# LiChaiUSTC/Speech-enhancement-based-on-a-maximum-likelihood-criterion

Measured on AMD Instinct MI355X. Metric: training frames/sec (128-frame minibatch), higher is better.
Workload: dtype f32

## Files before the change

### speech-enhancement-based-on-a-maximum-likelihood-criterion_amd/csrc/engine.hip

```cpp
#include <hip/hip_runtime.h>
#include <hip/hip_ext.h>

#include <dlfcn.h>
#include <math.h>
#include <stdarg.h>
#include <stdio.h>
#include <stdlib.h>
#include <string.h>

#include <functional>
#include <mutex>
#include <string>
#include <vector>

#include "../../include/mlggd.h"
#include "kernels.hip.h"
#include "spectral.hip.h"
#include "score.hip.h"

static thread_local char g_err[1024] = "";
static int fail(int code, const char *fmt, ...) {
    va_list ap;
    va_start(ap, fmt);
    vsnprintf(g_err, sizeof(g_err), fmt, ap);
// ... 127 lines not shown
    int device = 0;
    hipStream_t stream = nullptr, comm_stream = nullptr;
    hipStream_t dw_stream = nullptr;
    hipEvent_t ev_dx[MLGGD_MAXLAYER] = {0}, ev_upd = nullptr;
    int two_streams = 0;

    float *W[MLGGD_MAXLAYER] = {0}, *dW[MLGGD_MAXLAYER] = {0};
    float *bias[MLGGD_MAXLAYER] = {0}, *dbias[MLGGD_MAXLAYER] = {0};
    float *G[MLGGD_MAXLAYER] = {0}, *gb[MLGGD_MAXLAYER] = {0};
    float *gb_all = nullptr;
    size_t gb_all_count = 0;
    float *Gpre[MLGGD_MAXLAYER] = {0}, *gbpre = nullptr, *colsum_tot = nullptr;
    float *Yt[MLGGD_MAXLAYER] = {0}, *Y[MLGGD_MAXLAYER] = {0};
    float *dEdXt[MLGGD_MAXLAYER] = {0}, *dEdX[MLGGD_MAXLAYER] = {0};
    float *slab = nullptr, *outT = nullptr, *eT = nullptr, *pT = nullptr, *colsum = nullptr, *scalefactor = nullptr;
    int S_out = 1;
    float *chunk_in = nullptr, *chunk_targ = nullptr, *chunk_out = nullptr;
    int cv_device = 0;
    double *cv_partial = nullptr;
    size_t cv_partial_cap = 0;
    size_t chunk_cap = 0, out_cap = 0;
    int chunk_frames = 0;
    float *raw_feat = nullptr, *raw_targ = nullptr, *in_bunch = nullptr;
    float *in_bunch_buf[2] = {nullptr, nullptr};
    int *first_frame = nullptr;
    size_t raw_cap = 0, first_cap = 0;
    struct RawSet {
        float *feat = nullptr, *targ = nullptr;
        int *first = nullptr;
        size_t raw_cap = 0, first_cap = 0;
        hipEvent_t last_use = nullptr;
    } raw[2];
    int raw_cur = 0;
    hipStream_t copy_stream = nullptr;
    struct WsBuf {
        void *p = nullptr;
        size_t cap = 0;
    };
    struct WavesWs {
        WsBuf wave, lps, X, blk, out_i, out_f, lps_den, norm, frame_off, out_off, wave_off, utt_of;
        WsBuf clean, Xc, fstat, sframes, scores;
        std::vector<int32_t> h_frame_off, h_utt_of;
        std::vector<long long> h_out_off, h_wave_off;
        std::vector<float> h_norm;
        std::vector<float> h_scores;
        int lookup_table = 0;
    } ww;
    bool indexed = false;
    int fdim = 0, toff = 0, raw_frames = 0;
    unsigned step_counter = 0;
    int fwd_pipe = 4, dx_pipe = 4;
    int tile64 = 1, n_cus = 256;
    int fwd_nw = 4, dx_nw = 4, dw_tile = 1, dw_persist = 1, dwp_per_cu = 2, dw_merge = 1, loss_fuse = 1, tile_map = 0, stage_ahead = 1;

    int world = 1, rank = 0;
    int dp_mode = 0;
    int shard_rows[MLGGD_MAXLAYER] = {0};
    int dp_a2a = 0;
    std::vector<float *> Ysrc[MLGGD_MAXLAYER];
    hipEvent_t ev_W[MLGGD_MAXLAYER] = {0}, ev_dw_done = nullptr;
    bool ev_W_pending[MLGGD_MAXLAYER] = {false};
    bool fake_world = false;
    float *Yall[MLGGD_MAXLAYER] = {0}, *dEdXall[MLGGD_MAXLAYER] = {0};
    bool keep_ranks = false;
    std::vector<float *> snap_x, snap_out, snap_y[MLGGD_MAXLAYER], snap_dedx[MLGGD_MAXLAYER];
    hipEvent_t ev_ready = nullptr, ev_gathered = nullptr;
    int dp_fine = 1;
    hipEvent_t ev_layer[MLGGD_MAXLAYER] = {0};
    int dp_mainline = 1;
    bool comm_after_dw = false;
    RcclComm comm = nullptr;
    RcclComm stat_comm = nullptr;
    int ar_shard = 1;
    hipEvent_t ev_grad[MLGGD_MAXLAYER] = {0}, ev_red[MLGGD_MAXLAYER] = {0}, ev_bias = nullptr, ev_bias_red = nullptr;

    hipEvent_t ev_t0 = nullptr, ev_t1 = nullptr;
    int last_steps = 0;
    bool timing_valid = false;
    int prof_class = -1, prof_layer = 0, prof_stride = 1;
    std::vector<hipEvent_t> prof_ev;
    size_t prof_used = 0, prof_cap = 0;
    hipEvent_t *prof_attach = nullptr;
    bool prof_attached = false;
    hipEvent_t stop_ev_next = nullptr;
    bool stop_ev_attached = false;
    int dp_stopev = 1;
    double prof_flops = 0, prof_bytes = 0;

    int stamp_class = -1, stamp_layer = 0, stamp_blocks = 0;
    long long *stamp_buf = nullptr;
    size_t stamp_cap = 0;

    struct DwpTable {
        DwpJobs key;
        bool fused;
        int grid;
        DwpDesc *dev;
    };
    std::vector<DwpTable> dwp_tables;
    std::vector<void *> allocs;
    std::vector<const void *> lds_attr_done;
};

static long long *stamps_for(mlggd_engine *e, int cls, int layer, int blocks) {
    if (e->stamp_class != cls || e->stamp_layer != layer || !e->stamp_buf) return nullptr;
    if ((size_t)blocks * 8 > e->stamp_cap) return nullptr;
// ... 756 lines not shown
    CHK(launch_check("k_loss_err"));
    const float *colsum_in = nullptr;
    if (ML == 1 && cs == CS_GIVEN) {
        colsum_in = e->colsum_tot;
    } else if (ML == 1 && cs != CS_LOCAL) {
        hipLaunchKernelGGL(k_colsum, dim3(e->Dp / 32), dim3(256), 0, e->stream, e->pT, B, Bp, e->colsum);
        CHK(launch_check("k_colsum"));
        if (cs == CS_ACCUMULATE) {
            hipLaunchKernelGGL(k_accum, dim3(1), dim3(256), 0, e->stream, e->colsum_tot,
                               first_acc ? (const float *)nullptr : (const float *)e->colsum_tot, (const float *)e->colsum,
                               (size_t)e->Dp);
            return launch_check("k_accum");
        }
        NCCLCHK(g_rccl.AllReduce(e->colsum, e->colsum, (size_t)e->Dp, 7, 0, e->stat_comm ? e->stat_comm : e->comm, e->stream));
        colsum_in = e->colsum;
    }
    if (cs == CS_ACCUMULATE) return MLGGD_OK;
    CHK(ensure_lds(e, k_loss_grad, LOSS_LDS_MAX));
    hipLaunchKernelGGL(k_loss_grad, dim3(n_loss), dim3(256), lds_grad, e->stream, e->eT, e->pT, colsum_in, B, e->D, e->Dp, Bp,
                       e->cfg.shapefactor, ML, nf, inv_n, e->scalefactor, e->dEdXt[L - 1], e->dEdX[L - 1], b_tiles);
    return launch_check("k_loss_grad");
}

static int run_dx(mlggd_engine *e, int l) {
    const int Kp = e->lsp[l - 1], b_tiles = e->Bp / 32;
    ProfScope ps(e, KC_DX, l);
    DxArgs xa = dx_args(e, l);
    if (dx64_used(e, l)) {
        xa.k_tiles = Kp / 64;
        xa.b_tiles = e->Bp / 64;
        xa.b_shift = log2_or_minus1(xa.b_tiles);
        const size_t lds = t64_lds_floats() * sizeof(float);
        CHK(ensure_lds(e, k_dx64, lds));
        launch_timed(e, k_dx64, dim3(xa.k_tiles * xa.b_tiles), dim3(256), lds, e->stream, xa);
        return launch_check("k_dx64");
    }
    long long *st = stamps_for(e, KC_DX, l, (Kp / 32) * b_tiles);
#define LAUNCH_DX(NW, PIPE)                                                                                  \
    {                                                                                                        \
        const size_t lds = dx_lds_floats<NW, PIPE>() * sizeof(float);                                        \
        CHK(ensure_lds(e, k_dx<NW, PIPE>, lds));                                                             \
        launch_timed(e, k_dx<NW, PIPE>, dim3((Kp / 32) * b_tiles), dim3(64 * NW), lds, e->stream, xa, st);      \
    }
    const bool dma = e->dx_pipe == 4 && (Kp / 32) * b_tiles <= 256;
    if (e->dx_nw == 8 && e->dx_pipe) LAUNCH_DX(8, 1)
    else if (e->dx_nw == 8) LAUNCH_DX(8, 0)
    else if (dma) LAUNCH_DX(4, 4)
    else if (e->dx_pipe) LAUNCH_DX(4, 1)
    else LAUNCH_DX(4, 0)
#undef LAUNCH_DX
    return launch_check("k_dx");
}

static int launch_dw_layer(mlggd_engine *e, int l, const float *in_rows, bool fused, float nf, hipStream_t st) {
    const int Kp = e->lsp[l - 1], Np = e->lsp[l];
    const long tiles128 = (long)((Kp + 127) / 128) * ((Np + 127) / 128);
    const bool big = e->dw_tile == 0 ? tiles128 >= 192 : e->dw_tile == 2;
    ProfScope ps(e, KC_DW, l, st);
    if (dwp_usable(e)) return launch_dwp(e, dwp_jobs(e, l, l, in_rows, nf), fused, st, l);
    if (big) return launch_dw<2>(e, l, in_rows, fused, nf, st);
    return launch_dw<1>(e, l, in_rows, fused, nf, st);
}

static int launch_accum(float *dst, const float *a, const float *b, size_t n, hipStream_t st) {
    const size_t blocks = (n + 255) / 256;
    hipLaunchKernelGGL(k_accum, dim3((unsigned)(blocks > 2048 ? 2048 : blocks)), dim3(256), 0, st, dst, a, b, n);
    return launch_check("k_accum");
}

static size_t y_count(const mlggd_engine *e, int l) {
    return e->dp_a2a ? (size_t)e->world * e->Bp * e->shard_rows[l + 1] * 64 : (size_t)e->Bp * e->lsp[l];
}
static int keep_alloc(mlggd_engine *e) {
    if (!e->keep_ranks || !e->fake_world || !e->snap_x.empty()) return MLGGD_OK;
    for (int r = 0; r + 1 < e->world; r++) {
        float *p = nullptr;
        CHK(dev_alloc(e, &p, y_count(e, 0)));
        e->snap_x.push_back(p);
        CHK(dev_alloc(e, &p, (size_t)e->Dp * e->Bp));
        e->snap_out.push_back(p);
        for (int l = 1; l < e->L; l++) {
            if (l < e->L - 1) {
                CHK(dev_alloc(e, &p, y_count(e, l)));
                e->snap_y[l].push_back(p);
            }
            CHK(dev_alloc(e, &p, (size_t)e->Bp * e->lsp[l]));
            e->snap_dedx[l].push_back(p);
        }
    }
    HIPCHK(hipStreamSynchronize(e->stream));
    return MLGGD_OK;
}
static int keep_snapshot(mlggd_engine *e, int r, const float *in_rows) {
    auto cp = [&](float *dst, const float *src, size_t count) -> int {
        HIPCHK(hipMemcpyAsync(dst, src, count * sizeof(float), hipMemcpyDeviceToDevice, e->stream));
        return MLGGD_OK;
    };
    CHK(cp(e->snap_x[r], in_rows, y_count(e, 0)));
    CHK(cp(e->snap_out[r], e->outT, (size_t)e->Dp * e->Bp));
    for (int l = 1; l < e->L; l++) {
        if (l < e->L - 1) CHK(cp(e->snap_y[l][r], e->Y[l], y_count(e, l)));
        CHK(cp(e->snap_dedx[l][r], e->dEdX[l], (size_t)e->Bp * e->lsp[l]));
    }
    return MLGGD_OK;
}

// ... 21 lines not shown
            };
            if (e->dp_a2a) {
                for (int l = 0; l < L - 1; l++) {
                    const size_t all = (size_t)e->world * Bp * e->shard_rows[l + 1] * 64;
                    HIPCHK(hipMemcpyAsync(e->Ysrc[l][r], l == 0 ? in_rows : e->Y[l], all * sizeof(float), hipMemcpyDeviceToDevice, e->stream));
                }
            } else {
                CHK(put(in_rows, e->Yall[0], (size_t)Bp * e->lsp[0]));
                for (int l = 1; l < L - 1; l++) CHK(put(e->Y[l], e->Yall[l], (size_t)Bp * e->lsp[l]));
            }
            for (int l = 1; l < L; l++) CHK(put(e->dEdX[l], e->dEdXall[l], (size_t)Bp * e->lsp[l]));
        } else {
            for (int l = L - 1; l >= 1; l--) {
                CHK(launch_dw_layer(e, l, in_rows, false, nf, e->stream));
                CHK(launch_accum(e->Gpre[l], r == 0 ? nullptr : e->Gpre[l], e->G[l], (size_t)e->lsp[l - 1] * e->lsp[l], e->stream));
            }
            CHK(launch_accum(e->gbpre, r == 0 ? nullptr : e->gbpre, e->gb_all, e->gb_all_count, e->stream));
        }
    }
    return MLGGD_OK;
}

static int run_step(mlggd_engine *e, int sample0, bool prestaged = false, const Bunch *next = nullptr) {
    const int L = e->L, B = e->B, Bp = e->Bp;
    e->stop_ev_next = nullptr;
    e->stop_ev_attached = false;
    const bool dp = e->comm != nullptr || e->fake_world;
    const bool gather = dp && e->dp_mode >= 1;
    const int n_global = B * e->world;
    const float nf = (float)n_global;
    const float inv_n = 1.0f / n_global;
    const int ML = e->cfg.MLflag;
    if (e->fake_world) {
        CHK(fake_world_prepass(e, sample0, nf, inv_n));
        sample0 += (e->world - 1) * B;
    }
    const Bunch bn = bunch_at(e, sample0);
    RoctxRange step_range("mlggd step");

    const bool fine = gather && e->dp_mode == 1 && e->dp_fine != 0;
    {
        RoctxRange r("forward");
        CHK(run_forward(e, bn, B, true, prestaged,
                        gather ? (GATHER_INPUT | (ML != 1 ? (fine ? GATHER_HIDDEN_EACH : GATHER_HIDDEN) : 0)) : 0));
    }
    const float *in_rows = bunch_rows(e, bn);
    StageArgs sa;
    memset(&sa, 0, sizeof(sa));
    int n_stage = 0;
    if (next) {
        sa = stage_args(e, *next, B, in_bunch_other(e));
        n_stage = stage_blocks(e);
    }
    {
        RoctxRange r("loss (+ staging of the next minibatch)");
        CHK(run_loss(e, bn, nf, inv_n, !dp ? CS_LOCAL : e->fake_world ? CS_GIVEN : CS_ALLREDUCE, false, sa, n_stage));
    }
    RoctxRange back_range("backward: dX, dW + update, exchange");
    if (gather && ML == 1 && L > 2) {
        CHK(gather_begin(e));
        for (int g = 1; g < L - 1; g++) CHK(exchange_y(e, g, e->Y[g], nullptr));
        CHK(gather_end(e));
    }
    const bool two = e->two_streams != 0;
    hipStream_t dws = two ? e->dw_stream : e->stream;
    const bool merged = (!dp && !two && e->dw_merge && dwp_usable(e)) || gather;
    int pending_hi = L - 1;
    bool mainline_done = false;
    for (int l = L - 1; l >= 1; l--) {
        const int Kp = e->lsp[l - 1], Np = e->lsp[l];
        if (fine) {
            CHK(gather_begin_armed(e));
            CHK(gather_one(e, e->dEdX[l], e->dEdXall[l], (size_t)Bp * e->lsp[l]));
            CHK(gather_end(e));
            HIPCHK(hipEventRecord(e->ev_layer[l], e->comm_stream));
        } else if (gather && l <= 2) {
            if (l == 1 && e->dp_mainline && !two) {
                HIPCHK(hipEventRecord(e->ev_gathered, e->comm_stream));
                HIPCHK(hipStreamWaitEvent(e->stream, e->ev_gathered, 0));
                if (!e->fake_world) NCCLCHK(g_rccl.GroupStart());
                for (int g = pending_hi; g >= l; g--)
                    CHK(gather_one(e, e->dEdX[g], e->dEdXall[g], (size_t)Bp * e->lsp[g], e->stream));
                if (!e->fake_world) NCCLCHK(g_rccl.GroupEnd());
                mainline_done = true;
            } else {
                CHK(gather_begin_armed(e));
                for (int g = pending_hi; g >= l; g--) CHK(gather_one(e, e->dEdX[g], e->dEdXall[g], (size_t)Bp * e->lsp[g]));
                CHK(gather_end(e));
            }
            pending_hi = l - 1;
        }
        if (l != 1 && gather && !two &&
            (fine || l - 1 == 2 || (l - 1 == 1 && !(e->dp_mainline))))
            gather_arm(e);
        if (l != 1) CHK(run_dx(e, l));
        if (two) {
            HIPCHK(hipEventRecord(e->ev_dx[l], e->stream));
            HIPCHK(hipStreamWaitEvent(dws, e->ev_dx[l], 0));
        }
        if (merged) continue;
        if (dp && !gather && !two) arm_stop(e, e->ev_grad[l]);
        CHK(launch_dw_layer(e, l, in_rows, !dp, nf, dws));
        if (dp && !gather) {
            if (!take_stop(e)) HIPCHK(hipEventRecord(e->ev_grad[l], dws));
            HIPCHK(hipStreamWaitEvent(e->comm_stream, e->ev_grad[l], 0));
            if (e->fake_world) {
                if (e->world > 1) CHK(launch_accum(e->G[l], e->Gpre[l], e->G[l], (size_t)Kp * Np, e->comm_stream));
            } else if (e->ar_shard) {
                const size_t blk = (size_t)e->shard_rows[l] * 64 * Np;
                NCCLCHK(g_rccl.ReduceScatter(e->G[l], e->G[l] + (size_t)e->rank * blk, blk, e->comm, e->comm_stream));
            } else {
                NCCLCHK(g_rccl.AllReduce(e->G[l], e->G[l], (size_t)Kp * Np, 7, 0, e->comm, e->comm_stream));
            }
            HIPCHK(hipEventRecord(e->ev_red[l], e->comm_stream));
        }
    }
    if (gather && e->dp_mode == 2) {
        if (!mainline_done) {
            HIPCHK(hipEventRecord(e->ev_gathered, e->comm_stream));
            HIPCHK(hipStreamWaitEvent(dws, e->ev_gathered, 0));
        }
        const int units = e->world * Bp / 64;
        if (e->fake_world) {
            const char *only = getenv("MLGGD_FAKE_ONLY_RANK");
            for (int r = 0; r < e->world; r++) {
                if (only && atoi(only) != r) continue;
                if (e->dp_a2a)
                    for (int l = 0; l < L - 1; l++) {
                        const size_t cnt = (size_t)Bp * e->shard_rows[l + 1] * 64;
                        for (int sr = 0; sr < e->world; sr++) {
                            const float *src = sr + 1 < e->world ? e->Ysrc[l][sr] : (l == 0 ? in_rows : e->Y[l]);
                            HIPCHK(hipMemcpyAsync(e->Yall[l] + (size_t)sr * cnt, src + (size_t)r * cnt, cnt * sizeof(float),
                                                  hipMemcpyDeviceToDevice, dws));
                        }
                    }
                if (only || r == e->world - 1) {
                    DwpJobs Jb = dwp_jobs_shard(e, nf, r, 1, false);
                    if (Jb.total > 0) CHK(launch_dwp(e, Jb, true, dws, 1, units));
                }
                DwpJobs J = dwp_jobs_shard(e, nf, r, 0, only ? true : e->world == 1);
                ProfScope ps(e, KC_DW, 1, dws);
                if (J.total > 0) CHK(launch_dwp(e, J, true, dws, 1, units));
            }
        } else {
            {
                DwpJobs Jb = dwp_jobs_shard(e, nf, e->rank, 1, false);
                if (Jb.total > 0) CHK(launch_dwp(e, Jb, true, dws, 1, units));
                ProfScope ps(e, KC_DW, 1, dws);
// ... 107 lines not shown

int mlggd_create(const mlggd_config *cfg, const float *const *weights, const float *const *bias, mlggd_handle *out) {
    if (!cfg || !weights || !bias || !out) return fail(MLGGD_ERR_ARG, "NULL argument");
    if (cfg->struct_size != (int32_t)sizeof(mlggd_config))
        return fail(MLGGD_ERR_ARG, "mlggd_config.struct_size %d != %d", cfg->struct_size, (int)sizeof(mlggd_config));
    if (cfg->numlayers < 2 || cfg->numlayers > MLGGD_MAXLAYER)
        return fail(MLGGD_ERR_ARG, "numlayers %d not in 2..%d", cfg->numlayers, MLGGD_MAXLAYER);
    if (cfg->bunchsize < 1) return fail(MLGGD_ERR_ARG, "bunchsize %d < 1", cfg->bunchsize);
    for (int i = 0; i < cfg->numlayers; i++)
        if (cfg->layersizes[i] < 1) return fail(MLGGD_ERR_ARG, "layersizes[%d] = %d", i, cfg->layersizes[i]);
    for (int i = 1; i < cfg->numlayers; i++) {
        const long long bytes = 4ll * ceil32(cfg->layersizes[i - 1]) * ceil32(cfg->layersizes[i]);
        if (bytes >= (1ll << 31))
            return fail(MLGGD_ERR_ARG, "layer %d: %d x %d weights exceed the 2 GiB a kernel can address", i,
                        cfg->layersizes[i - 1], cfg->layersizes[i]);
    }
    if (ceil32(cfg->bunchsize) > 1152)
        return fail(MLGGD_ERR_ARG, "bunchsize %d too large for the loss kernel's LDS tile (max 1152)", cfg->bunchsize);
    int ndev = 0;
    hipError_t de = hipGetDeviceCount(&ndev);
    if (de != hipSuccess || ndev < 1)
        return fail(MLGGD_ERR_DEVICE, "no HIP device available (%s)", de == hipSuccess ? "count 0" : hipGetErrorString(de));
    if (cfg->device < 0 || cfg->device >= ndev)
        return fail(MLGGD_ERR_ARG, "GPU Num %d Not In Range %d-%d", cfg->device, 0, ndev - 1);

    mlggd_engine *e = new mlggd_engine();
    e->cfg = *cfg;
    e->L = cfg->numlayers;
    e->device = cfg->device;
    for (int i = 0; i < e->L; i++) {
        e->ls[i] = cfg->layersizes[i];
        e->lsp[i] = ceil32(cfg->layersizes[i]);
    }
    e->B = cfg->bunchsize;
    e->Bp = ceil32(e->B);
    e->K0 = e->ls[0];
    e->D = e->ls[e->L - 1];
    e->Dp = e->lsp[e->L - 1];
    if (const char *v = getenv("MLGGD_FWD_NW")) e->fwd_nw = atoi(v);
    if (const char *v = getenv("MLGGD_WAVES_LOOKUP")) e->ww.lookup_table = !strcmp(v, "table");
    if (const char *v = getenv("MLGGD_DX_NW")) e->dx_nw = atoi(v);
    if (const char *v = getenv("MLGGD_FWD_PIPE")) e->fwd_pipe = atoi(v);
    if (const char *v = getenv("MLGGD_DX_PIPE")) e->dx_pipe = atoi(v);
    if (const char *v = getenv("MLGGD_DW_TILE")) e->dw_tile = atoi(v);
    if (const char *v = getenv("MLGGD_TWO_STREAMS")) e->two_streams = atoi(v);
    if (const char *v = getenv("MLGGD_DW_PERSIST")) e->dw_persist = atoi(v);
    if (const char *v = getenv("MLGGD_DWP_PER_CU")) e->dwp_per_cu = atoi(v);
    if (const char *v = getenv("MLGGD_DW_MERGE")) e->dw_merge = atoi(v);
    if (const char *v = getenv("MLGGD_LOSS_FUSE")) e->loss_fuse = atoi(v);
    if (const char *v = getenv("MLGGD_TILE_MAP")) e->tile_map = atoi(v);
    if (const char *v = getenv("MLGGD_STAGE_AHEAD")) e->stage_ahead = atoi(v);
    if (const char *v = getenv("MLGGD_CV_DEVICE")) e->cv_device = atoi(v) ? 1 : 0;
    if (const char *v = getenv("MLGGD_TILE64")) e->tile64 = atoi(v);
    *out = e;

    roctx_load();
    HIPCHK(hipSetDevice(e->device));
    {
        int cus = 0;
        if (hipDeviceGetAttribute(&cus, hipDeviceAttributeMultiprocessorCount, e->device) == hipSuccess && cus > 0) e->n_cus = cus;
    }
    HIPCHK(hipStreamCreateWithFlags(&e->stream, hipStreamNonBlocking));
    if (e->two_streams) HIPCHK(hipStreamCreateWithFlags(&e->dw_stream, hipStreamNonBlocking));
    for (int l = 0; l < e->L; l++) HIPCHK(hipEventCreateWithFlags(&e->ev_dx[l], hipEventDisableTiming));
    HIPCHK(hipEventCreateWithFlags(&e->ev_upd, hipEventDisableTiming));
    HIPCHK(hipEventCreate(&e->ev_t0));
    HIPCHK(hipEventCreate(&e->ev_t1));

    const int L = e->L, Bp = e->Bp;
    CHK(dev_alloc(e, &e->Yt[0], (size_t)e->lsp[0] * Bp));
    CHK(dev_alloc(e, &e->in_bunch_buf[0], (size_t)(Bp + 1) * e->lsp[0]));
    CHK(dev_alloc(e, &e->in_bunch_buf[1], (size_t)(Bp + 1) * e->lsp[0]));
    e->in_bunch = e->in_bunch_buf[0];
    for (int l = 1; l < L; l++) {
        const size_t wsz = (size_t)e->lsp[l - 1] * e->lsp[l];
        CHK(dev_alloc(e, &e->W[l], wsz));
        CHK(dev_alloc(e, &e->dW[l], wsz));
        CHK(dev_alloc(e, &e->bias[l], e->lsp[l]));
        CHK(dev_alloc(e, &e->dbias[l], e->lsp[l]));
        const size_t asz = (size_t)e->lsp[l] * Bp;
        if (l != L - 1) {
            CHK(dev_alloc(e, &e->Yt[l], asz));
            CHK(dev_alloc(e, &e->Y[l], asz));
        }
        CHK(dev_alloc(e, &e->dEdXt[l], asz));
        CHK(dev_alloc(e, &e->dEdX[l], asz));
    }
    {
        const int tiles = (e->Dp / 32) * (Bp / 32);
        const int pairs = e->lsp[L - 2] / 2;
        int S = 256 / tiles >= 4 ? 256 / tiles : (256 + tiles - 1) / tiles;
        if (S > pairs / 16) S = pairs / 16;
        if (S < 1) S = 1;
        if (S > 32) S = 32;
        if (const char *v = getenv("MLGGD_S_OUT")) S = atoi(v) < 1 ? 1 : atoi(v) > 32 ? 32 : atoi(v);
        e->S_out = S;
    }
    CHK(dev_alloc(e, &e->slab, (size_t)e->S_out * e->Dp * Bp));
    CHK(dev_alloc(e, &e->outT, (size_t)e->Dp * Bp));
    CHK(dev_alloc(e, &e->eT, (size_t)e->Dp * Bp));
    CHK(dev_alloc(e, &e->pT, (size_t)e->Dp * Bp));
    CHK(dev_alloc(e, &e->colsum, e->Dp));
    CHK(dev_alloc(e, &e->scalefactor, e->Dp));

    const int rc = mlggd_set_weights(e, weights, bias);
    if (rc != MLGGD_OK) return rc;
// ... 508 lines not shown
    HIPCHK(hipStreamSynchronize(e->stream));
    return MLGGD_OK;
}

static int rows_to_host(mlggd_engine *e, const float *src, int N, int Np, int yb, float *dst) {
    const int B = e->B, Bp = e->Bp;
    std::vector<float> t(yb ? (size_t)e->world * Bp * yb : (size_t)Bp * Np);
    HIPCHK(hipMemcpyAsync(t.data(), src, t.size() * 4, hipMemcpyDeviceToHost, e->stream));
    HIPCHK(hipStreamSynchronize(e->stream));
    for (int b = 0; b < B; b++)
        for (int n = 0; n < N; n++)
            dst[(size_t)b * N + n] = yb ? t[(size_t)(n / yb) * Bp * yb + (size_t)b * yb + n % yb] : t[(size_t)b * Np + n];
    return MLGGD_OK;
}
static int out_to_host(mlggd_engine *e, const float *outT, float *dst) {
    std::vector<float> t((size_t)e->Dp * e->Bp);
    HIPCHK(hipMemcpyAsync(t.data(), outT, t.size() * 4, hipMemcpyDeviceToHost, e->stream));
    HIPCHK(hipStreamSynchronize(e->stream));
    for (int b = 0; b < e->B; b++)
        for (int d = 0; d < e->D; d++) dst[(size_t)b * e->D + d] = t[(size_t)d * e->Bp + b];
    return MLGGD_OK;
}

int mlggd_debug_tensor(mlggd_handle e, const char *name, int layer, float *dst, size_t count) {
    if (!e || !name || !dst) return fail(MLGGD_ERR_ARG, "NULL argument");
    HIPCHK(hipSetDevice(e->device));
    const int L = e->L, B = e->B, Bp = e->Bp;
    const std::string nm(name);
    auto need = [&](size_t n) -> int {
        return count < n ? fail(MLGGD_ERR_ARG, "dst holds %zu floats, %s needs %zu", count, name, n) : MLGGD_OK;
    };
    if (nm == "scalefactor") {
        CHK(need(e->D));
        return mlggd_get_scalefactor(e, dst);
    }
    if (nm == "out") {
        CHK(need((size_t)B * e->D));
        return out_to_host(e, e->outT, dst);
    }
    if (layer < 1 || layer >= L) return fail(MLGGD_ERR_ARG, "layer %d not in 1..%d", layer, L - 1);
    const int N = e->ls[layer], Np = e->lsp[layer], K = e->ls[layer - 1];
    if (nm == "y" || nm == "dedx" || nm == "yt" || nm == "dedxt") {
        const bool tr = (nm == "yt" || nm == "dedxt");
        const float *src = (nm == "y") ? e->Y[layer] : (nm == "dedx") ? e->dEdX[layer]
                           : (nm == "yt") ? e->Yt[layer] : e->dEdXt[layer];
        if (!src) return fail(MLGGD_ERR_ARG, "%s not kept for layer %d", name, layer);
        CHK(need((size_t)B * N));
        if (!tr) return rows_to_host(e, src, N, Np, (nm == "y" && e->dp_a2a && layer < L - 1) ? e->shard_rows[layer + 1] * 64 : 0, dst);
        std::vector<float> t((size_t)Np * Bp);
        HIPCHK(hipMemcpyAsync(t.data(), src, t.size() * 4, hipMemcpyDeviceToHost, e->stream));
        HIPCHK(hipStreamSynchronize(e->stream));
        for (int b = 0; b < B; b++)
            for (int n = 0; n < N; n++) dst[(size_t)b * N + n] = t[(size_t)n * Bp + b];
        return MLGGD_OK;
    }
    if (nm == "weights" || nm == "delta_w" || nm == "grad_w") {
        CHK(wait_weight_gathers(e, 1, L - 1));
        const float *src = (nm == "weights") ? e->W[layer] : (nm == "delta_w") ? e->dW[layer] : e->G[layer];
        if (!src) return fail(MLGGD_ERR_STATE, "tensor %s does not exist on this path", name);
        if (!src) return fail(MLGGD_ERR_ARG, "%s not kept for layer %d", name, layer);
        CHK(need((size_t)K * N));
        CHK(download_padded(dst, src, Np, K, N, e->stream));
        HIPCHK(hipStreamSynchronize(e->stream));
        return MLGGD_OK;
    }
    if (nm == "bias" || nm == "delta_b") {
        CHK(need(N));
        HIPCHK(hipMemcpyAsync(dst, nm == "bias" ? e->bias[layer] : e->dbias[layer], (size_t)N * 4,
                              hipMemcpyDeviceToHost, e->stream));
        HIPCHK(hipStreamSynchronize(e->stream));
        return MLGGD_OK;
    }
    return fail(MLGGD_ERR_ARG, "unknown tensor name '%s'", name);
}

int mlggd_debug_keep_ranks(mlggd_handle e, int on) {
    if (!e) return fail(MLGGD_ERR_ARG, "NULL handle");
    HIPCHK(hipSetDevice(e->device));
    e->keep_ranks = on != 0;
    return keep_alloc(e);
}

int mlggd_debug_rank_tensor(mlggd_handle e, const char *name, int layer, int rank, float *dst, size_t count) {
    if (!e || !name || !dst) return fail(MLGGD_ERR_ARG, "NULL argument");
    HIPCHK(hipSetDevice(e->device));
    const int L = e->L, B = e->B;
    const std::string nm(name);
    if (rank < 0 || rank >= e->world) return fail(MLGGD_ERR_ARG, "rank %d not in 0..%d", rank, e->world - 1);
    const bool live = rank == (e->fake_world ? e->world - 1 : e->rank);
    if (!live && (!e->fake_world || (size_t)rank >= e->snap_x.size()))
        return fail(MLGGD_ERR_STATE, "rank %d: only emulated ranks are kept (mlggd_debug_keep_ranks before training)", rank);
    auto need = [&](size_t n) -> int {
        return count < n ? fail(MLGGD_ERR_ARG, "dst holds %zu floats, %s needs %zu", count, name, n) : MLGGD_OK;
    };
    if (nm == "out") {
        CHK(need((size_t)B * e->D));
        return out_to_host(e, live ? e->outT : e->snap_out[rank], dst);
    }
    if (nm == "x") {
        CHK(need((size_t)B * e->ls[0]));
        return rows_to_host(e, live ? e->in_bunch : e->snap_x[rank], e->ls[0], e->lsp[0], e->dp_a2a ? e->shard_rows[1] * 64 : 0, dst);
    }
    if (nm == "y" || nm == "dedx") {
        const bool y = nm == "y";
        if (layer < 1 || layer >= (y ? L - 1 : L)) return fail(MLGGD_ERR_ARG, "%s: layer %d not in 1..%d", name, layer, y ? L - 2 : L - 1);
        CHK(need((size_t)B * e->ls[layer]));
// ... 294 lines not shown
    for (auto &x : ev) HIPCHK(hipEventCreate(&x));
    auto nop = [&]() -> int {
        hipLaunchKernelGGL(k_nop, dim3(256), dim3(256), 0, e->stream);
        return launch_check("k_nop");
    };
    for (int r = 0; r < reps; r++) {
        HIPCHK(hipEventRecord(ev[4 * r], e->stream));
        CHK(nop());
        HIPCHK(hipEventRecord(ev[4 * r + 1], e->stream));
        HIPCHK(hipEventRecord(ev[4 * r + 2], e->stream));
        CHK(nop());
        CHK(nop());
        HIPCHK(hipEventRecord(ev[4 * r + 3], e->stream));
    }
    HIPCHK(hipStreamSynchronize(e->stream));
    double t1 = 0, t2 = 0;
    for (int r = 4; r < reps; r++) {
        float a = 0, b = 0;
        HIPCHK(hipEventElapsedTime(&a, ev[4 * r], ev[4 * r + 1]));
        HIPCHK(hipEventElapsedTime(&b, ev[4 * r + 2], ev[4 * r + 3]));
        t1 += a;
        t2 += b;
    }
    for (auto &x : ev) hipEventDestroy(x);
    const double ov = (2 * t1 - t2) / (reps - 4) * 1000.0;
    *usec = ov > 0 ? (float)ov : 0.0f;
    return MLGGD_OK;
}

int mlggd_dw_launches_per_step(mlggd_handle e, int *launches) {
    if (!e || !launches) return fail(MLGGD_ERR_ARG, "NULL argument");
    const bool dp = e->comm != nullptr || e->fake_world;
    const bool merged = (!dp && !e->two_streams && e->dw_merge && dwp_usable(e)) || (dp && e->dp_mode >= 1);
    const bool fine = dp && e->dp_mode == 1 && e->dp_fine != 0 && e->L - 1 >= 2;
    *launches = fine ? 2 : merged ? 1 : e->L - 1;
    return MLGGD_OK;
}

int mlggd_kernel_work(mlggd_handle e, const char *kernel_class, int layer, double *flops, double *bytes) {
    if (!e || !kernel_class) return fail(MLGGD_ERR_ARG, "NULL argument");
    double f = 0, by = 0;
    const bool dpx = (e->comm != nullptr || e->fake_world) && e->dp_mode >= 1 && !strcmp(kernel_class, "dw");
    const double W = e->world, B = e->B;
    auto gemm = [&](const char *cls, int l, double &ff, double &bb) {
        if (l < 1 || l >= e->L) return;
        const double K = e->ls[l - 1], N = e->ls[l];
        if (!strcmp(cls, "fwd")) {
            ff += 2.0 * B * K * N;
            bb += 4.0 * (K * N + B * K + 2 * B * N);
        } else if (!strcmp(cls, "dx")) {
            if (l == 1) return;
            ff += 2.0 * B * K * N;
            bb += 4.0 * (K * N + B * N + 3 * B * K);
        } else if (!strcmp(cls, "dw")) {
            if (!dpx) {
                ff += 2.0 * B * K * N;
                bb += 4.0 * (4 * K * N + B * K + B * N);
            } else if (e->dp_mode == 1) {
                ff += 2.0 * B * W * K * N;
                bb += 4.0 * (4 * K * N + B * W * K + B * W * N);
            } else {
                ff += 2.0 * B * W * K * N / W;
                bb += 4.0 * (4 * K * N / W + B * W * K / W + B * W * N);
            }
        }
    };
    for (int l = 1; l < e->L; l++) {
        if (layer != 0 && layer != l) continue;
        gemm(kernel_class, l, f, by);
    }
    if (flops) *flops = f;
    if (bytes) *bytes = by;
    return MLGGD_OK;
}

}

namespace {

struct SpecPlan {
    SpecDims d;
    float *win = nullptr;
    float2 *tw = nullptr;
    float2 *tws = nullptr;
};
constexpr int SPEC_MAX_DEVICES = 64;
std::mutex g_spec_mu;
SpecPlan g_spec[SPEC_MAX_DEVICES][3];

int spec_dims(int fs_khz, SpecDims *d, int *slot) {
    int L, S, N;
    switch (fs_khz) {
        case 8: L = 256, S = 128, N = 256, *slot = 0; break;
        case 11: L = 256, S = 110, N = 256, *slot = 1; break;
        case 16: L = 512, S = 256, N = 512, *slot = 2; break;
        default: return fail(MLGGD_ERR_ARG, "fs_khz %d: must be 8, 11 or 16", fs_khz);
    }
    d->L = L, d->S = S, d->N = N, d->M = N / 2, d->D = N / 2 + 1;
    d->logM = 0;
    while ((1 << d->logM) < d->M) d->logM++;
    return MLGGD_OK;
}

float2 twiddle(int k, int n) {
    const double a = -2.0 * M_PI * k / n;
    double c = cos(a), s = sin(a);
// ... 531 lines not shown
```

### speech-enhancement-based-on-a-maximum-likelihood-criterion_amd/csrc/kernels.hip.h

```cpp
#pragma once
#include <hip/hip_runtime.h>

typedef float f32x16 __attribute__((ext_vector_type(16)));
typedef float f32x2 __attribute__((ext_vector_type(2)));

__device__ __forceinline__ f32x16 mfma32(float a, float b, f32x16 c) {
    return __builtin_amdgcn_mfma_f32_32x32x2f32(a, b, c, 0, 0, 0);
}
__device__ __forceinline__ int acc_row(int r, int lane) { return (r & 3) + 8 * (r >> 2) + 4 * (lane >> 5); }

__device__ __forceinline__ void divmod_by(int x, int d, int shift, int &q, int &r) {
    if (shift >= 0) {
        q = x >> shift;
        r = x & (d - 1);
    } else {
        q = (int)((unsigned)x / (unsigned)d);
        r = x - q * d;
    }
}
__device__ __forceinline__ void tile_of_block(int id, int u_tiles, int b_tiles, int b_shift, int &ut, int &bt, int map = 0) {
    if ((u_tiles & 7) == 0 && map != 2) {
        const int xcd = id & 7, slot = id >> 3;
        int q;
        divmod_by(slot, b_tiles, b_shift, q, bt);
// ... 1450 lines not shown
    jb.bias[n] = d + 1.0f * bv;
}

struct StageArgs {
    const float *in;
    int ld, B, K, Kp;
    float *inT;
    int Bp, b_tiles;
    const int *first;
    int fdim;
    float *rows_out;
    int yblk;
};
template <int SUB = 1>
__device__ __forceinline__ void transpose_in_body(const StageArgs &A, const int bid, const int n_tiles = 0x7FFFFFFF) {
    const float *__restrict__ in = A.in;
    float *__restrict__ inT = A.inT, *__restrict__ rows_out = A.rows_out;
    const int *__restrict__ first = A.first;
    const int ld = A.ld, B = A.B, K = A.K, Bp = A.Bp, b_tiles = A.b_tiles, fdim = A.fdim;
    __shared__ float ts[SUB][32][33];
    const int sub = SUB == 1 ? 0 : (int)(threadIdx.x >> 8), tile = SUB * bid + sub;
    float(*t)[33] = ts[sub];
    const bool live = tile < n_tiles;
    const int kt = tile / b_tiles, bt = tile % b_tiles;
    const int k0 = kt * 32, b0 = bt * 32;
    const int tx = threadIdx.x & 31, ty = (threadIdx.x >> 5) & 7;
    if (live) {
#pragma unroll
        for (int q = 0; q < 4; q++) {
            const int b = b0 + ty + 8 * q, k = k0 + tx;
            float v = 0.0f;
            if (b < B && k < K) {
                const size_t base = first ? (size_t)first[b] * fdim : (size_t)b * ld;
                v = in[base + k];
            }
            if (rows_out) {
                if (A.yblk) rows_out[y_blocked_base(k0, A.yblk, Bp) + (size_t)b * A.yblk + tx] = v;
                else rows_out[(size_t)b * A.Kp + k] = v;
            }
            t[ty + 8 * q][tx] = v;
        }
    }
    __syncthreads();
    if (live) {
#pragma unroll
        for (int q = 0; q < 4; q++) {
            const int k = k0 + ty + 8 * q;
            inT[(size_t)k * Bp + b0 + tx] = t[tx][ty + 8 * q];
        }
    }
}
__global__ __launch_bounds__(256) void k_transpose_in(StageArgs A) { transpose_in_body(A, (int)blockIdx.x); }

__device__ __forceinline__ float slab_sum(const float *__restrict__ slab, size_t o, size_t stride, int S) {
    float v[8];
#pragma unroll
    for (int s = 0; s < 8; s++) v[s] = slab[(size_t)(s < S ? s : 0) * stride + o];
    float x = v[0];
#pragma unroll
    for (int s = 1; s < 8; s++)
        if (s < S) x += v[s];
    for (int s = 8; s < S; s++) x += slab[(size_t)s * stride + o];
    return x;
}

constexpr int LOSS_DT = 8;
__device__ __forceinline__ float pow_or_self(float x, float p) { return p == 1.0f ? x : p == 0.0f ? 1.0f : pow_det(x, p); }

struct LossErrArgs {
    const float *slab;
    int S;
    const float *bias, *targ;
    int B, D, Dp, Bp;
    float beta;
    int want_pow;
    float *outT, *eT, *pT;
    int b_tiles;
    const int *first;
    int toff;
};
__device__ __forceinline__ void loss_err_body(const LossErrArgs &A, const int bid) {
    const float *__restrict__ slab = A.slab, *__restrict__ bias = A.bias, *__restrict__ targ = A.targ;
    float *__restrict__ outT = A.outT, *__restrict__ eT = A.eT, *__restrict__ pT = A.pT;
    const int *__restrict__ first = A.first;
    const int dt = bid / A.b_tiles, bt = bid % A.b_tiles;
    const int d = dt * LOSS_DT + (int)(threadIdx.x >> 5), b = bt * 32 + (int)(threadIdx.x & 31);
    const size_t o = (size_t)d * A.Bp + b;
    float x = slab_sum(slab, o, (size_t)A.Dp * A.Bp, A.S);
    x = x + bias[d];
    float e = 0.0f, p = 0.0f;
    if (b < A.B && d < A.D) {
        e = x - targ[(size_t)(first ? first[b] + A.toff : b) * A.D + d];
        if (A.want_pow) p = pow_or_self(fabsf(e), A.beta);
    } else {
        x = 0.0f;
    }
    outT[o] = x;
    eT[o] = e;
    pT[o] = p;
}
__global__ __launch_bounds__(256) void k_loss_err(LossErrArgs A, int n_loss, StageArgs G) {
    const int n_stage = (int)gridDim.x - n_loss;
    if ((int)blockIdx.x >= n_stage) loss_err_body(A, (int)blockIdx.x - n_stage);
    else transpose_in_body(G, (int)blockIdx.x);
}

template <int DT>
__device__ __forceinline__ void colsum_tile(const float *__restrict__ pT, int d0, int B, int Bp, float *rows,
                                            float *sums) {
    const int total = DT * Bp;
    for (int idx = threadIdx.x; idx < total; idx += 256) {
        const int dl = idx / Bp, b = idx - dl * Bp;
        rows[dl * (Bp + 1) + b] = pT[(size_t)(d0 + dl) * Bp + b];
    }
// ... 43 lines not shown
    if (MLflag == 1) {
        float *rows = dyn, *sums = dyn + LOSS_DT * (Bp + 1);
        if (colsum_in == nullptr) {
            colsum_tile<LOSS_DT>(pT, d0, B, Bp, rows, sums);
        } else {
            if (tid < LOSS_DT) sums[tid] = colsum_in[d0 + tid];
            __syncthreads();
        }
        if (tid < LOSS_DT) {
            const int d = d0 + tid;
            float q = 1.0f;
            if (d < D) {
                const float v1 = sums[tid] / nf;
                const float v2 = v1 * beta;
                const float alpha = pow_or_self(v2, 1.0f / beta);
                if (bt == 0) scalefactor[d] = alpha;
                q = pow_or_self(alpha, beta);
            }
            denom[tid] = q;
        }
        __syncthreads();
    }
    const int dl = tid >> 5, d = d0 + dl, b = bt * 32 + (tid & 31);
    const size_t o = (size_t)d * Bp + b;
    const float e = eT[o];
    float g = 0.0f;
    if (b < B && d < D) {
        if (MLflag == 1) {
            if (e > 0) g = pow_or_self(e, beta - 1.0f) * beta / denom[dl];
            else if (e == 0) g = 0;
            else g = -pow_or_self(-e, beta - 1.0f) * beta / denom[dl];
        } else {
            if (e > 0) g = beta * pow_or_self(e, beta - 1);
            else if (e == 0) g = 0;
            else g = -beta * pow_or_self(-e, beta - 1);
        }
        g = g * inv_n;
    }
    dEdXt[o] = g;
    dEdX[(size_t)b * Dp + d] = g;
}

struct LossNormArgs {
    const float *slab;
    int S;
    const float *bias, *targ;
    int B, D, Dp, Bp;
    float beta, inv_n;
    float *outT, *eT, *dEdXt, *dEdX;
    int b_tiles;
    const int *first;
    int toff;
};
__device__ __forceinline__ void loss_norm_body(const LossNormArgs &A, const int bid) {
    const float *__restrict__ slab = A.slab, *__restrict__ bias = A.bias, *__restrict__ targ = A.targ;
    float *__restrict__ outT = A.outT, *__restrict__ eT = A.eT, *__restrict__ dEdXt = A.dEdXt, *__restrict__ dEdX = A.dEdX;
    const int *__restrict__ first = A.first;
    const float beta = A.beta;
    const int dt = bid / A.b_tiles, bt = bid % A.b_tiles;
    const int d = dt * LOSS_DT + (int)(threadIdx.x >> 5), b = bt * 32 + (int)(threadIdx.x & 31);
    const size_t o = (size_t)d * A.Bp + b;
    float x = slab_sum(slab, o, (size_t)A.Dp * A.Bp, A.S);
    x = x + bias[d];
    float e = 0.0f, g = 0.0f;
    if (b < A.B && d < A.D) {
        e = x - targ[(size_t)(first ? first[b] + A.toff : b) * A.D + d];
        if (e > 0) g = beta * pow_or_self(e, beta - 1);
        else if (e == 0) g = 0;
        else g = -beta * pow_or_self(-e, beta - 1);
        g = g * A.inv_n;
    } else {
        x = 0.0f;
    }
    outT[o] = x;
    eT[o] = e;
    dEdXt[o] = g;
    dEdX[(size_t)b * A.Dp + d] = g;
}
__global__ __launch_bounds__(256) void k_loss_norm(LossNormArgs A, int n_loss, StageArgs G) {
    const int n_stage = (int)gridDim.x - n_loss;
    if ((int)blockIdx.x >= n_stage) loss_norm_body(A, (int)blockIdx.x - n_stage);
    else transpose_in_body(G, (int)blockIdx.x);
}

struct LossMlArgs {
    const float *slab;
    int S;
    const float *bias, *targ;
    int B, D, Dp, Bp;
    float beta, nf, inv_n;
    float *outT, *eT, *scalefactor, *dEdXt, *dEdX;
    const int *first;
    int toff;
};
__global__ __launch_bounds__(1024) void k_loss_ml(LossMlArgs A, int n_loss, StageArgs G, int n_stage_tiles) {
    const int n_stage = (int)gridDim.x - n_loss;
    if ((int)blockIdx.x < n_stage) {
        transpose_in_body<4>(G, (int)blockIdx.x, n_stage_tiles);
        return;
    }
    extern __shared__ __attribute__((aligned(16))) float dyn[];
    __shared__ float denom[LOSS_DT];
    const float *__restrict__ slab = A.slab, *__restrict__ bias = A.bias, *__restrict__ targ = A.targ;
    const int *__restrict__ first = A.first;
    const int B = A.B, D = A.D, Dp = A.Dp, Bp = A.Bp;
    const float beta = A.beta;
    float *es = dyn, *ps = dyn + LOSS_DT * (Bp + 1);
    const int d0 = ((int)blockIdx.x - n_stage) * LOSS_DT;
    const int tid = threadIdx.x, dl = tid >> 7, d = d0 + dl;
    for (int b = tid & 127; b < Bp; b += 128) {
        const size_t o = (size_t)d * Bp + b;
        float x = slab_sum(slab, o, (size_t)Dp * Bp, A.S);
        x = x + bias[d];
        float e = 0.0f, p = 0.0f;
        if (b < B && d < D) {
            e = x - targ[(size_t)(first ? first[b] + A.toff : b) * D + d];
            p = pow_or_self(fabsf(e), beta);
        } else {
            x = 0.0f;
        }
        A.outT[o] = x;
        A.eT[o] = e;
        es[dl * (Bp + 1) + b] = e;
        ps[dl * (Bp + 1) + b] = p;
    }
    __syncthreads();
    if (tid < LOSS_DT) {
        const float *col = ps + tid * (Bp + 1);
        float s = col[0];
        int b = 1;
        for (; b + 16 <= B; b += 16) {
            float v[16];
#pragma unroll
            for (int u = 0; u < 16; u++) v[u] = col[b + u];
#pragma unroll
// ... 140 lines not shown
```

Before: 1.019 million.

## Fold normalized loss computation into the last-layer dX kernel

Adds a k_dxl kernel that recomputes the loss gradient (slab sum, bias, error, pow gradient) for its N-strip directly into LDS and consumes it in the dX MFMA for the top layer. This removes the separate loss kernel launch and the global round trip of dEdXt between loss and dX. Only the kt==0 blocks write outT/eT/dEdXt/dEdX for later use, and staging blocks for the next minibatch ride along in the same grid. The cost is redundant loss recomputation across k-tiles and extra slab reads, and the path is limited to non-ML, beta in {1,2}, single-stream, small-shape configurations.

```diff
diff --git a/speech-enhancement-based-on-a-maximum-likelihood-criterion_amd/csrc/engine.hip b/speech-enhancement-based-on-a-maximum-likelihood-criterion_amd/csrc/engine.hip
--- a/speech-enhancement-based-on-a-maximum-likelihood-criterion_amd/csrc/engine.hip
+++ b/speech-enhancement-based-on-a-maximum-likelihood-criterion_amd/csrc/engine.hip
@@ -203,6 +203,7 @@
     int fwd_pipe = 4, dx_pipe = 4;
     int tile64 = 1, n_cus = 256;
     int fwd_nw = 4, dx_nw = 4, dw_tile = 1, dw_persist = 1, dwp_per_cu = 2, dw_merge = 1, loss_fuse = 1, tile_map = 0, stage_ahead = 1;
+    int loss_fold = 1;
 
     int world = 1, rank = 0;
     int dp_mode = 0;
@@ -1065,6 +1066,30 @@
     return launch_check("k_dx");
 }
 
+static bool loss_fold_used(const mlggd_engine *e) {
+    const int L = e->L;
+    const float p = e->cfg.shapefactor - 1;
+    if (!e->loss_fold || e->comm != nullptr || e->fake_world || e->two_streams) return false;
+    if (e->cfg.MLflag == 1 || !e->loss_fuse || L < 3 || !(p == 1.0f || p == 0.0f)) return false;
+    if (e->dx_pipe != 4 || e->dx_nw != 4 || dx64_used(e, L - 1) || (e->lsp[L - 2] / 32) * (e->Bp / 32) > 256) return false;
+    return e->Dp <= DXL_MAX_NP && e->S_out <= DXL_MAX_S;
+}
+static int run_dx_fold(mlggd_engine *e, const Bunch &bn, float inv_n, const StageArgs &sa, int n_stage) {
+    const int L = e->L, Bp = e->Bp, b_tiles = Bp / 32, n_dx = (e->lsp[L - 2] / 32) * b_tiles;
+    ProfScope ps(e, KC_DX, L - 1);
+    DxArgs xa = dx_args(e, L - 1);
+    LossNormArgs la;
+    la.slab = e->slab; la.S = e->S_out; la.bias = e->bias[L - 1]; la.targ = bn.targ;
+    la.B = e->B; la.D = e->D; la.Dp = e->Dp; la.Bp = Bp; la.beta = e->cfg.shapefactor; la.inv_n = inv_n;
+    la.outT = e->outT; la.eT = e->eT; la.dEdXt = e->dEdXt[L - 1]; la.dEdX = e->dEdX[L - 1];
+    la.b_tiles = b_tiles; la.first = bn.first; la.toff = e->toff;
+    long long *st = stamps_for(e, KC_DX, L - 1, n_dx);
+    const size_t lds = dxl_lds_floats() * sizeof(float);
+    CHK(ensure_lds(e, k_dxl, lds));
+    launch_timed(e, k_dxl, dim3(n_dx + n_stage), dim3(256), lds, e->stream, xa, la, n_dx, sa, st);
+    return launch_check("k_dxl");
+}
+
 static int launch_dw_layer(mlggd_engine *e, int l, const float *in_rows, bool fused, float nf, hipStream_t st) {
     const int Kp = e->lsp[l - 1], Np = e->lsp[l];
     const long tiles128 = (long)((Kp + 127) / 128) * ((Np + 127) / 128);
@@ -1192,7 +1217,8 @@
         sa = stage_args(e, *next, B, in_bunch_other(e));
         n_stage = stage_blocks(e);
     }
-    {
+    const bool fold = loss_fold_used(e);
+    if (!fold) {
         RoctxRange r("loss (+ staging of the next minibatch)");
         CHK(run_loss(e, bn, nf, inv_n, !dp ? CS_LOCAL : e->fake_world ? CS_GIVEN : CS_ALLREDUCE, false, sa, n_stage));
     }
@@ -1233,7 +1259,7 @@
         if (l != 1 && gather && !two &&
             (fine || l - 1 == 2 || (l - 1 == 1 && !(e->dp_mainline))))
             gather_arm(e);
-        if (l != 1) CHK(run_dx(e, l));
+        if (l != 1) CHK(fold && l == L - 1 ? run_dx_fold(e, bn, inv_n, sa, n_stage) : run_dx(e, l));
         if (two) {
             HIPCHK(hipEventRecord(e->ev_dx[l], e->stream));
             HIPCHK(hipStreamWaitEvent(dws, e->ev_dx[l], 0));
@@ -1447,6 +1473,7 @@
     if (const char *v = getenv("MLGGD_STAGE_AHEAD")) e->stage_ahead = atoi(v);
     if (const char *v = getenv("MLGGD_CV_DEVICE")) e->cv_device = atoi(v) ? 1 : 0;
     if (const char *v = getenv("MLGGD_TILE64")) e->tile64 = atoi(v);
+    if (const char *v = getenv("MLGGD_LOSS_FOLD")) e->loss_fold = atoi(v) ? 1 : 0;
     *out = e;
 
     roctx_load();
@@ -2061,6 +2088,15 @@
         HIPCHK(hipStreamSynchronize(e->stream));
         for (int b = 0; b < B; b++)
             for (int n = 0; n < N; n++) dst[(size_t)b * N + n] = t[(size_t)n * Bp + b];
+        return MLGGD_OK;
+    }
+    if (nm == "raw_et" || nm == "raw_dedx" || nm == "raw_dedxt") {
+        const float *src = nm == "raw_et" ? e->eT : nm == "raw_dedx" ? e->dEdX[layer] : e->dEdXt[layer];
+        const size_t n = (size_t)(nm == "raw_et" ? e->Dp : Np) * Bp;
+        if (!src) return fail(MLGGD_ERR_ARG, "%s not kept for layer %d", name, layer);
+        CHK(need(n));
+        HIPCHK(hipMemcpyAsync(dst, src, n * 4, hipMemcpyDeviceToHost, e->stream));
+        HIPCHK(hipStreamSynchronize(e->stream));
         return MLGGD_OK;
     }
     if (nm == "weights" || nm == "delta_w" || nm == "grad_w") {
@@ -2461,6 +2497,7 @@
             if (l == 1) return;
             ff += 2.0 * B * K * N;
             bb += 4.0 * (K * N + B * N + 3 * B * K);
+            if (l == e->L - 1 && loss_fold_used(e)) bb += 4.0 * ((e->S_out + 4) * B * N + N);
         } else if (!strcmp(cls, "dw")) {
             if (!dpx) {
                 ff += 2.0 * B * K * N;
diff --git a/speech-enhancement-based-on-a-maximum-likelihood-criterion_amd/csrc/kernels.hip.h b/speech-enhancement-based-on-a-maximum-likelihood-criterion_amd/csrc/kernels.hip.h
--- a/speech-enhancement-based-on-a-maximum-likelihood-criterion_amd/csrc/kernels.hip.h
+++ b/speech-enhancement-based-on-a-maximum-likelihood-criterion_amd/csrc/kernels.hip.h
@@ -1526,14 +1526,18 @@
 }
 __global__ __launch_bounds__(256) void k_transpose_in(StageArgs A) { transpose_in_body(A, (int)blockIdx.x); }
 
+__device__ __forceinline__ float slab_add8(const float *v, int S) {
+    float x = v[0];
+#pragma unroll
+    for (int s = 1; s < 8; s++)
+        if (s < S) x += v[s];
+    return x;
+}
 __device__ __forceinline__ float slab_sum(const float *__restrict__ slab, size_t o, size_t stride, int S) {
     float v[8];
 #pragma unroll
     for (int s = 0; s < 8; s++) v[s] = slab[(size_t)(s < S ? s : 0) * stride + o];
-    float x = v[0];
-#pragma unroll
-    for (int s = 1; s < 8; s++)
-        if (s < S) x += v[s];
+    float x = slab_add8(v, S);
     for (int s = 8; s < S; s++) x += slab[(size_t)s * stride + o];
     return x;
 }
@@ -1683,6 +1687,21 @@
     const int *first;
     int toff;
 };
+__device__ __forceinline__ void loss_norm_elem(float &x, float bias, bool live, float t, float beta, float inv_n, float &e,
+                                               float &g) {
+    x = x + bias;
+    e = 0.0f;
+    g = 0.0f;
+    if (live) {
+        e = x - t;
+        if (e > 0) g = beta * pow_or_self(e, beta - 1);
+        else if (e == 0) g = 0;
+        else g = -beta * pow_or_self(-e, beta - 1);
+        g = g * inv_n;
+    } else {
+        x = 0.0f;
+    }
+}
 __device__ __forceinline__ void loss_norm_body(const LossNormArgs &A, const int bid) {
     const float *__restrict__ slab = A.slab, *__restrict__ bias = A.bias, *__restrict__ targ = A.targ;
     float *__restrict__ outT = A.outT, *__restrict__ eT = A.eT, *__restrict__ dEdXt = A.dEdXt, *__restrict__ dEdX = A.dEdX;
@@ -1691,18 +1710,10 @@
     const int dt = bid / A.b_tiles, bt = bid % A.b_tiles;
     const int d = dt * LOSS_DT + (int)(threadIdx.x >> 5), b = bt * 32 + (int)(threadIdx.x & 31);
     const size_t o = (size_t)d * A.Bp + b;
-    float x = slab_sum(slab, o, (size_t)A.Dp * A.Bp, A.S);
-    x = x + bias[d];
-    float e = 0.0f, g = 0.0f;
-    if (b < A.B && d < A.D) {
-        e = x - targ[(size_t)(first ? first[b] + A.toff : b) * A.D + d];
-        if (e > 0) g = beta * pow_or_self(e, beta - 1);
-        else if (e == 0) g = 0;
-        else g = -beta * pow_or_self(-e, beta - 1);
-        g = g * A.inv_n;
-    } else {
-        x = 0.0f;
-    }
+    const bool live = b < A.B && d < A.D;
+    const float t = live ? targ[(size_t)(first ? first[b] + A.toff : b) * A.D + d] : 0.0f;
+    float x = slab_sum(slab, o, (size_t)A.Dp * A.Bp, A.S), e, g;
+    loss_norm_elem(x, bias[d], live, t, beta, A.inv_n, e, g);
     outT[o] = x;
     eT[o] = e;
     dEdXt[o] = g;
@@ -1712,6 +1723,153 @@
     const int n_stage = (int)gridDim.x - n_loss;
     if ((int)blockIdx.x >= n_stage) loss_norm_body(A, (int)blockIdx.x - n_stage);
     else transpose_in_body(G, (int)blockIdx.x);
+}
+
+constexpr int dxl_lds_floats() { return 4 * 8192 + 32 * 36; }
+constexpr int DXL_MAX_NP = 512, DXL_MAX_S = 8;
+
+__device__ __forceinline__ void dxl_body(const DxArgs &A, const LossNormArgs &Lo, const int bid, float *smem, long long *stamps) {
+    constexpr int NW = 4;
+    const float *__restrict__ W = A.W, *__restrict__ Yt_prev = A.Yt_prev;
+    float *__restrict__ dEdXt_prev = A.dEdXt_prev, *__restrict__ dEdX_prev = A.dEdX_prev;
+    const int Kp = A.Kp, Np = A.Np, Bp = A.Bp, k_tiles = A.k_tiles, b_tiles = A.b_tiles;
+    float(*tileT)[36] = reinterpret_cast<float(*)[36]>(smem + NW * 8192);
+    stamp(stamps, 0, bid);
+    const int tid = threadIdx.x, lane = tid & 63, wave = wave_id();
+    const int i = lane & 31, h = lane >> 5;
+    int kt, bt;
+    tile_of_block(bid, k_tiles, b_tiles, A.b_shift, kt, bt, A.map);
+    const int k0 = kt * 32, b0 = bt * 32;
+
+    const int Q = Np >> 2;
+    const int qw = (Q + NW - 1) / NW;
+    const int q0 = wave * qw;
+    const int qend = (q0 + qw < Q) ? q0 + qw : Q;
+    const int myq = qend > q0 ? qend - q0 : 0;
+    const int nch = (myq + 15) >> 4;
+
+    float *ws0 = smem + wave * 8192, *ws1 = ws0 + 2048, *strip = ws0 + 4096;
+    const rsrc_t rW = make_rsrc(W, (size_t)Kp * Np * 4);
+
+    f32x16 acc;
+#pragma unroll
+    for (int r = 0; r < 16; r++) acc[r] = 0.0f;
+    const float4 y_pre4 = *reinterpret_cast<const float4 *>(&Yt_prev[(size_t)(k0 + (tid >> 3)) * Bp + b0 + (tid & 7) * 4]);
+    asm volatile("" ::: "memory");
+
+    const int endW = Kp * Np * 4;
+    const int wr = lane >> 4, wq = lane & 15;
+    int voWd[4];
+#pragma unroll
+    for (int tt = 0; tt < 4; tt++) voWd[tt] = ((k0 + wr) * Np + 4 * (wq ^ (4 * tt + wr))) * 4;
+#pragma unroll
+    for (int c = 0; c < 2; c++) {
+        float *ws = c == 0 ? ws0 : ws1;
+        const bool live = c < nch;
+        const int quad0 = q0 + c * 16;
+#pragma unroll
+        for (int t = 0; t < 8; t++)
+            __builtin_amdgcn_raw_ptr_buffer_load_lds(rW, (__attribute__((address_space(3))) void *)(ws + t * 256), 16,
+                                                     voWd[t & 3], live ? quad0 * 16 + t * (16 * Np) : endW, 0, 0);
+    }
+
+    {
+        const float *__restrict__ slab = Lo.slab, *__restrict__ bias = Lo.bias, *__restrict__ targ = Lo.targ;
+        const int *__restrict__ first = Lo.first;
+        const int S = Lo.S, B = Lo.B, D = Lo.D;
+        const size_t sstride = (size_t)Np * Bp;
+        const float beta = Lo.beta, inv_n = Lo.inv_n;
+        const int r8 = lane >> 3, c4 = lane & 7;
+        const int b = b0 + 4 * c4;
+        const bool side = kt == 0;
+        size_t trow[4];
+#pragma unroll
+        for (int t = 0; t < 4; t++) trow[t] = (b + t < B) ? (size_t)(first ? first[b + t] + Lo.toff : b + t) * D : 0;
+#pragma unroll 2
+        for (int it = 0; it < myq >> 1; it++) {
+            const int lr = it * 8 + r8, n = 4 * q0 + lr;
+            const size_t o = (size_t)n * Bp + b;
+            float4 v[8];
+#pragma unroll
+            for (int s = 0; s < 8; s++) v[s] = *reinterpret_cast<const float4 *>(&slab[(size_t)(s < S ? s : 0) * sstride + o]);
+            const float bn = bias[n];
+            float tv[4], x[4], e[4], g[4];
+#pragma unroll
+            for (int t = 0; t < 4; t++) tv[t] = (b + t < B && n < D) ? targ[trow[t] + n] : 0.0f;
+#pragma unroll
+            for (int t = 0; t < 4; t++) {
+                float vs[8];
+#pragma unroll
+                for (int s = 0; s < 8; s++) vs[s] = t == 0 ? v[s].x : t == 1 ? v[s].y : t == 2 ? v[s].z : v[s].w;
+                x[t] = slab_add8(vs, S);
+                loss_norm_elem(x[t], bn, b + t < B && n < D, tv[t], beta, inv_n, e[t], g[t]);
+            }
+            const int w = lr & 63, pos = (lr & ~63) | (w & ~3) | ((w & 1) << 1) | ((w >> 1) & 1);
+            *reinterpret_cast<float4 *>(strip + pos * 32 + 4 * c4) = make_float4(g[0], g[1], g[2], g[3]);
+            if (side) {
+                *reinterpret_cast<float4 *>(&Lo.outT[o]) = make_float4(x[0], x[1], x[2], x[3]);
+                *reinterpret_cast<float4 *>(&Lo.eT[o]) = make_float4(e[0], e[1], e[2], e[3]);
+                *reinterpret_cast<float4 *>(&Lo.dEdXt[o]) = make_float4(g[0], g[1], g[2], g[3]);
+#pragma unroll
+                for (int t = 0; t < 4; t++) Lo.dEdX[(size_t)(b + t) * Np + n] = g[t];
+            }
+        }
+    }
+    __builtin_amdgcn_s_waitcnt(0x0F70);
+    asm volatile("" ::: "memory");
+    __builtin_amdgcn_wave_barrier();
+    __builtin_amdgcn_sched_barrier(0);
+
+#pragma unroll
+    for (int c = 0; c < 2; c++) {
+        const float *ws = c == 0 ? ws0 : ws1, *ds = strip + c * 2048;
+        const int cnt = myq - 16 * c;
+#pragma unroll
+        for (int j = 0; j < 16; j++) {
+            if (j < cnt) {
+                const int ao = i * 64 + 4 * (j ^ (i & 15)) + 2 * h;
+                const float2 av = *reinterpret_cast<const float2 *>(ws + ao);
+                acc = mfma32(av.x, ds[h * 32 + i + (4 * j) * 32], acc);
+                acc = mfma32(av.y, ds[h * 32 + i + (4 * j + 2) * 32], acc);
+            }
+        }
+    }
+
+    stamp(stamps, 1, bid);
+    __syncthreads();
+    float(*red)[1024] = reinterpret_cast<float(*)[1024]>(smem);
+#pragma unroll
+    for (int r = 0; r < 16; r++) red[wave][acc_row(r, lane) * 32 + i] = acc[r];
+    __syncthreads();
+    stamp(stamps, 2, bid);
+    const int row = tid >> 3, col4 = (tid & 7) * 4;
+    float4 d4 = *reinterpret_cast<const float4 *>(&red[0][row * 32 + col4]);
+#pragma unroll
+    for (int w = 1; w < NW; w++) {
+        const float4 p4 = *reinterpret_cast<const float4 *>(&red[w][row * 32 + col4]);
+        d4.x += p4.x;
+        d4.y += p4.y;
+        d4.z += p4.z;
+        d4.w += p4.w;
+    }
+    float4 g4;
+    g4.x = (1.0f - y_pre4.x) * y_pre4.x * d4.x;
+    g4.y = (1.0f - y_pre4.y) * y_pre4.y * d4.y;
+    g4.z = (1.0f - y_pre4.z) * y_pre4.z * d4.z;
+    g4.w = (1.0f - y_pre4.w) * y_pre4.w * d4.w;
+    *reinterpret_cast<float4 *>(&dEdXt_prev[(size_t)(k0 + row) * Bp + b0 + col4]) = g4;
+    tileT[col4][row] = g4.x;
+    tileT[col4 + 1][row] = g4.y;
+    tileT[col4 + 2][row] = g4.z;
+    tileT[col4 + 3][row] = g4.w;
+    __syncthreads();
+    *reinterpret_cast<float4 *>(&dEdX_prev[(size_t)(b0 + row) * Kp + k0 + col4]) =
+        *reinterpret_cast<const float4 *>(&tileT[row][col4]);
+    stamp(stamps, 3, bid);
+}
+__global__ __launch_bounds__(256) void k_dxl(DxArgs A, LossNormArgs Lo, int n_dx, StageArgs G, long long *stamps) {
+    if ((int)blockIdx.x < n_dx) dxl_body(A, Lo, (int)blockIdx.x, g_dyn_lds, stamps);
+    else transpose_in_body(G, (int)blockIdx.x - n_dx);
 }
 
 struct LossMlArgs {
```

New measurement: 930,700. -8.7%, worse.
